# farshid83/dpsvm

Hardware: AMD Instinct MI355X
Metric: wall-clock training time (s) to tol=1e-3, MNIST even-odd RBF, at 1/2/4/8 MI355X (lower is better)
Workload: dtype fp32

## Files before the change

### dpsvm_amd/csrc/kernels/rbf_gemm_split.hip

```cpp
#include <hip/hip_runtime.h>

#include <algorithm>
#include <cmath>
#include <cstdlib>
#include <map>
#include <mutex>
#include <string>
#include <tuple>
#include <vector>

#include "dpsvm/common.hpp"
#include "device_util.hpp"
#include "kernels.hpp"
#include "split_mma.hpp"
#include "../runtime/hip_check.hpp"

namespace dpsvm {
namespace dev {

constexpr int kSplitThreads = 512;
constexpr int kSplitShiftTarget = 15;

constexpr int kSplitRowChunks = 4;
__global__ __launch_bounds__(256) void split_rows_kernel(const float* __restrict__ x, int64_t rows, int dp, int ldx,
                                                         u4* __restrict__ out, int32_t* __restrict__ shift,
                                                         int nkb) {
  const int lane = threadIdx.x & 63;
  const int64_t r = (int64_t)blockIdx.x * 4 + (threadIdx.x >> 6);
// ... 571 lines not shown
        o[7] = t;
      }
    }
    if (!has_next) break;
    L = Ln;
    t = tn_next;
    par ^= 1;
    Ln = L + G;
    if (Ln < ntiles) tn_next = tiles[Ln];
  }
}
#undef PIECE_A
#undef PIECE_B
#undef ROW_DMA

__device__ __forceinline__ bool h1_values(f16v (&H)[2][2], const float* s_sq, const int32_t* s_sh, const float* s_r,
                                          int lane, int wm, int wn, float gamma, float c0, float c1) {
  constexpr int TM = 256;
  const int hl = lane >> 5;
  const float ng = -gamma, l2e = 1.4426950408889634f;
  bool hot = false;
#pragma unroll
  for (int j = 0; j < 2; ++j) {
    const int cl = wn * 64 + 32 * j + (lane & 31);
    const float bsq = s_sq[TM + cl];
    const int nbsh = -s_sh[TM + cl];
    const float rb = s_r[TM + cl];
#pragma unroll
    for (int i = 0; i < 2; ++i) {
      __builtin_amdgcn_sched_barrier(0);
      const int lr0 = wm * 64 + 32 * i + 4 * hl;
#pragma unroll
      for (int g = 0; g < 4; ++g) {
        const f4 asq = *(const f4*)(s_sq + lr0 + 8 * g);
        const i4v ash = *(const i4v*)(s_sh + lr0 + 8 * g);
        const f4 ar = *(const f4*)(s_r + lr0 + 8 * g);
#pragma unroll
        for (int e = 0; e < 4; e += 2) {
          const int r = 4 * g + e;
          f2 h, dot, sq, d2, t;
          h.x = H[i][j][r];
          h.y = H[i][j][r + 1];
          {
#pragma clang fp contract(off)
            dot.x = ldexpf(h.x, nbsh - ash[e]);
            dot.y = ldexpf(h.y, nbsh - ash[e + 1]);
            sq.x = asq[e];
            sq.y = asq[e + 1];
            d2 = (sq + bsq) - (dot + dot);
            d2.x = d2.x > 0.f ? d2.x : 0.f;
            d2.y = d2.y > 0.f ? d2.y : 0.f;
            t = (ng * d2) * l2e;
            hot |= !split_cold(t.x, ar[e] + rb, c0, c1);
            hot |= !split_cold(t.y, ar[e + 1] + rb, c0, c1);
          }
          H[i][j][r] = __builtin_amdgcn_exp2f(t.x);
          H[i][j][r + 1] = __builtin_amdgcn_exp2f(t.y);
        }
      }
    }
  }
  return __builtin_amdgcn_ballot_w64(hot) != 0;
}

__device__ __forceinline__ void h1_store_block(const f16v& v, int i, int j, int lane, int wm, int wn, bool mirror,
                                               bool valid, float* out, int m0, int n0, int M, int N, int ldo) {
  constexpr int TM = 256, TN = 128;
  constexpr uint32_t OOB = 0x80000000u;
  const int hl = lane >> 5;
  float* const ob = out + ((int64_t)m0 * ldo + n0);
  float* const mb = out + ((int64_t)n0 * ldo + m0);
  const uint32_t ld = (uint32_t)ldo;
  const int rlim = min(M - m0, TM);
  const int clim = min(N - n0, TN);
  const int64_t ob_bytes = min<int64_t>((int64_t)(M - m0) * ldo * 4 - (int64_t)n0 * 4, (int64_t)OOB);
  const int64_t mb_bytes = min<int64_t>((int64_t)(N - n0) * ldo * 4 - (int64_t)m0 * 4, (int64_t)OOB);
  const __amdgpu_buffer_rsrc_t rs_o = __builtin_amdgcn_make_buffer_rsrc(ob, 0, (int)ob_bytes, 0x00020000);
  const __amdgpu_buffer_rsrc_t rs_m = __builtin_amdgcn_make_buffer_rsrc(mb, 0, (int)mb_bytes, 0x00020000);
  const int cl = wn * 64 + 32 * j + (lane & 31);
  const bool okc = valid && cl < clim;
  constexpr int CP = 0;
  const int lr0 = wm * 64 + 32 * i + 4 * hl;
// ... 16 lines not shown
    w.z = v[4 * q + 2];
    w.w = v[4 * q + 3];
    const uint32_t o = lr + 3 < rlim && okm ? vm + 32u * q : OOB;
    __builtin_amdgcn_raw_buffer_store_b128(__builtin_bit_cast(i4v, w), rs_m, (int)o, 0, CP);
    if (rlim < TM) {
#pragma unroll
      for (int c = 0; c < 4; ++c) {
        const uint32_t oc = (okm && lr + 3 >= rlim && lr + c < rlim) ? vm + 32u * q + 4u * c : OOB;
        const float vc = w[c];
        __builtin_amdgcn_raw_buffer_store_b32(__float_as_uint(vc), rs_m, (int)oc, 0, CP);
      }
    }
  }
}

__device__ __forceinline__ uint32_t clock_lo_v() {
  uint32_t c = (uint32_t)__builtin_amdgcn_s_memtime();
  asm volatile("" : "+v"(c));
  return c;
}

template <bool ST>
__device__ __noinline__ void h1s_dma(const u4* __restrict__ A, const int32_t* __restrict__ Ash,
                                     const float* __restrict__ Asq, const float* __restrict__ Ar, int M,
                                     const u4* __restrict__ B, const int32_t* __restrict__ Bsh,
                                     const float* __restrict__ Bsq, const float* __restrict__ Br, int N, int nst,
                                     const uint32_t* __restrict__ tiles, int ntiles, int L, int dwave, int lane,
                                     u4* lds, uint32_t* s_rows, uint64_t* stamps) {
  constexpr int TM = 256, TN = 128, ROWS = TM + TN, NB = 3, RD = 1536;
  const int G = gridDim.x;
  const uint32_t rs = (uint32_t)nst * 8;
  uint32_t t = tiles[L];
  int Ln = L + G;
  uint32_t tn_next = Ln < ntiles ? tiles[Ln] : 0u;
  uint32_t g = 0;
  const int dw = __builtin_amdgcn_readfirstlane(dwave);
    const int p = lane & 7;
    uint32_t off_e = 16u * ((uint32_t)(lane >> 3) * rs + (uint32_t)(p ^ (lane >> 4)));
    uint32_t off_o = 16u * ((uint32_t)(lane >> 3) * rs + (uint32_t)(p ^ ((lane >> 4) + 4)));
    asm volatile("" : "+v"(off_e), "+v"(off_o));
    auto stage = [&](int m0_, int n0_, int st, int buf) {
      const uint32_t uA = (uint32_t)(m0_ + 64 * dw) * rs + (uint32_t)st * 8;
      const uint32_t uB = (uint32_t)(n0_ + 32 * dw) * rs + (uint32_t)st * 8;
#pragma unroll
      for (int i = 0; i < 8; ++i) w64p_piece(A, lds, uA, 8 * rs, 64 * dw * 8, off_e, off_o, buf, i);
#pragma unroll
      for (int i = 0; i < 4; ++i) w64p_piece(B, lds, uB, 8 * rs, (TM + 32 * dw) * 8, off_e, off_o, buf, i);
    };
    const uint32_t* const rd_a =
        dw == 0 ? (const uint32_t*)Asq : dw == 1 ? (const uint32_t*)Ash : (const uint32_t*)Ar;
    const uint32_t* const rd_b =
        dw == 0 ? (const uint32_t*)Bsq : dw == 1 ? (const uint32_t*)Bsh : (const uint32_t*)Br;
    auto rowdata = [&](int m0_, int n0_, int par_) {
#pragma unroll
      for (int i = 0; i < 6; ++i) {
        const int r = 64 * i + lane;
        const int ri = i < 4 ? min(m0_ + r, M - 1) : min(n0_ + (r - TM), N - 1);
        const uint32_t* src = dw == 3 ? (const uint32_t*)Asq : (i < 4 ? rd_a : rd_b) + ri;
        lds_dma4(src, s_rows + par_ * RD + 64 * (6 * dw + i));
      }
    };
    {
      const int m0 = (int)(t >> 16) * TM, n0 = (int)(t & 0xffffu) * TN;
      stage(m0, n0, 0, 0);
      stage(m0, n0, 1, 1);
      rowdata(m0, n0, 0);
      asm volatile("s_waitcnt vmcnt(0)" ::: "memory");
    }
    int par = 0;
    while (true) {
      const bool has_next = Ln < ntiles;
      const int m0 = (int)(t >> 16) * TM, n0 = (int)(t & 0xffffu) * TN;
      const uint32_t tp = has_next ? tn_next : t;
      const int nm0 = (int)(tp >> 16) * TM, nn0 = (int)(tp & 0xffffu) * TN;
      uint32_t c_bar0 = 0, c_bar = 0, c_land = 0, c_t0 = 0;
      if constexpr (ST) c_t0 = clock_lo_v();
#pragma clang loop unroll(disable)
      for (int s = 0; s < nst; ++s) {
        uint32_t ca = 0, cb = 0;
        if constexpr (ST) ca = clock_lo_v();
        if (s == 1) asm volatile("s_waitcnt vmcnt(18)" ::: "memory");
        else asm volatile("s_waitcnt vmcnt(12)" ::: "memory");
        if constexpr (ST) cb = clock_lo_v();
        __builtin_amdgcn_s_barrier();
        asm volatile("" ::: "memory");
        if constexpr (ST) {
          const uint32_t cc = clock_lo_v();
          c_land += cb - ca;
          if (s == 0) c_bar0 = cc - cb;
          else c_bar += cc - cb;
        }
        const bool own = s + 2 < nst;
        stage(own ? m0 : nm0, own ? n0 : nn0, own ? s + 2 : s + 2 - nst, (int)((g + 2) % NB));
        if (s == 0) rowdata(nm0, nn0, par ^ 1);
        ++g;
      }
      if constexpr (ST) {
        const uint32_t c_t1 = clock_lo_v();
        if (dw == 0 && lane == 0) {
          uint64_t* o = stamps + (size_t)L * 16 + 8;
          o[0] = c_bar0;
          o[1] = c_bar;
          o[2] = c_land;
          o[3] = c_t1 - c_t0;
        }
      }
      if (!has_next) break;
      L = Ln;
      t = tn_next;
      par ^= 1;
      Ln = L + G;
      if (Ln < ntiles) tn_next = tiles[Ln];
    }
  asm volatile("s_waitcnt vmcnt(0)" ::: "memory");
}

constexpr int kH1sThreads = 768;
template <bool ST>
__global__ __launch_bounds__(kH1sThreads, 1) void rbf_gemm_split_h1s_kernel(
    const u4* __restrict__ A, const int32_t* __restrict__ Ash, const float* __restrict__ Asq,
    const float* __restrict__ Ar, int M, const u4* __restrict__ B, const int32_t* __restrict__ Bsh,
    const float* __restrict__ Bsq, const float* __restrict__ Br, int N, int nkb, float gamma, float c0, float c1,
    float* __restrict__ out, int ldo, int sym, const uint32_t* __restrict__ tiles, int ntiles,
    uint32_t* __restrict__ tile_hot, uint32_t* __restrict__ hot, uint64_t* __restrict__ stamps) {
  constexpr int WN = 2, TM = 256, TN = 128, ROWS = TM + TN, CPR = 8, BUF = ROWS * CPR, NB = 3, RD = 1536;
  __shared__ u4 lds[NB * BUF + 2 * RD / 4];
  uint32_t* const s_rows = (uint32_t*)(lds + NB * BUF);
  const int G = gridDim.x;
  int L = blockIdx.x;
  if (L >= ntiles) return;
  const int tid = threadIdx.x, lane = tid & 63, wave = tid >> 6;
  const int nst = (nkb + 1) >> 1;
  if (__builtin_amdgcn_readfirstlane(wave) >= 8) {
    h1s_dma<ST>(A, Ash, Asq, Ar, M, B, Bsh, Bsq, Br, N, nst, tiles, ntiles, L, wave - 8, lane, lds, s_rows, stamps);
    return;
  }
  uint32_t t = tiles[L];
  int Ln = L + G;
  uint32_t tn_next = Ln < ntiles ? tiles[Ln] : 0u;
  uint32_t g = 0;
  const int wm = wave / WN, wn = wave % WN, hl = lane >> 5;
  const int sw = ((lane & 31) >> 1) & 7;
  const int ra0 = (wm * 64 + (lane & 31)) * CPR;
  const int rb0 = (TM + wn * 64 + (lane & 31)) * CPR;
  int par = 0;
  auto stamp = [&](int i, uint32_t v) {
    if (tid == 0) stamps[(size_t)L * 16 + i] = v;
  };
  while (true) {
    const bool has_next = Ln < ntiles;
    const int tx = (int)(t >> 16), ty = (int)(t & 0xffffu);
    const int m0 = tx * TM, n0 = ty * TN;
    if constexpr (ST) {
      stamp(0, (uint32_t)__builtin_amdgcn_s_memtime());
      stamp(5, (uint32_t)__builtin_amdgcn_s_memrealtime());
    }
    f16v H[2][2];
#pragma unroll
    for (int i = 0; i < 2; ++i)
#pragma unroll
      for (int j = 0; j < 2; ++j)
#pragma unroll
        for (int r = 0; r < 16; ++r) H[i][j][r] = 0.f;
    auto stage = [&]<bool FS = false>() {
      ring_barrier();
      if constexpr (ST && FS) stamp(1, (uint32_t)__builtin_amdgcn_s_memtime());
      const u4* buf = lds + (g % NB) * BUF;
      const uint32_t abase = lds_addr(buf + ra0), bbase = lds_addr(buf + rb0);
      auto rd = [&](int q, h8& a0, h8& a1, h8& b0, h8& b1) {
        const uint32_t c = 16u * (uint32_t)((2 * q + hl) ^ sw);
        const uint32_t pa = abase + c, pb = bbase + c;
        asm volatile("ds_read_b128 %0, %1" : "=v"(a0) : "v"(pa) : "memory");
        asm volatile("ds_read_b128 %0, %1 offset:4096" : "=v"(a1) : "v"(pa) : "memory");
        asm volatile("ds_read_b128 %0, %1" : "=v"(b0) : "v"(pb) : "memory");
        asm volatile("ds_read_b128 %0, %1 offset:4096" : "=v"(b1) : "v"(pb) : "memory");
      };
      auto mma = [&](const h8& a0, const h8& a1, const h8& b0, const h8& b1) {
        H[0][0] = mfma32_f16(a0, b0, H[0][0]);
        H[0][1] = mfma32_f16(a0, b1, H[0][1]);
        H[1][0] = mfma32_f16(a1, b0, H[1][0]);
        H[1][1] = mfma32_f16(a1, b1, H[1][1]);
      };
      h8 x0, x1, x2, x3, y0, y1, y2, y3;
      rd(0, x0, x1, x2, x3);
      rd(1, y0, y1, y2, y3);
      asm volatile("s_waitcnt lgkmcnt(4)" : "+v"(x0), "+v"(x1), "+v"(x2), "+v"(x3));
      mma(x0, x1, x2, x3);
      rd(2, x0, x1, x2, x3);
      asm volatile("s_waitcnt lgkmcnt(4)" : "+v"(y0), "+v"(y1), "+v"(y2), "+v"(y3));
      mma(y0, y1, y2, y3);
      rd(3, y0, y1, y2, y3);
      asm volatile("s_waitcnt lgkmcnt(4)" : "+v"(x0), "+v"(x1), "+v"(x2), "+v"(x3));
      mma(x0, x1, x2, x3);
      asm volatile("s_waitcnt lgkmcnt(0)" : "+v"(y0), "+v"(y1), "+v"(y2), "+v"(y3));
      mma(y0, y1, y2, y3);
      ++g;
    };
    if constexpr (ST) stage.template operator()<true>();
#pragma clang loop unroll(disable)
    for (int s = ST ? 1 : 0; s < nst; ++s) stage();
    if constexpr (ST) stamp(2, (uint32_t)__builtin_amdgcn_s_memtime());
    int el = lane;
    asm volatile("" : "+v"(el));
    const float* rows = (const float*)(s_rows + par * RD);
    const bool hotw = h1_values(H, rows, (const int32_t*)(rows + ROWS), rows + 2 * ROWS, el, wm, wn, gamma, c0, c1);
    if constexpr (ST) stamp(3, (uint32_t)__builtin_amdgcn_s_memtime());
    const bool mirror = sym && ty > 2 * tx + (wm >> 1);
#pragma unroll
    for (int i = 0; i < 2; ++i)
#pragma unroll
      for (int j = 0; j < 2; ++j) {
        __builtin_amdgcn_sched_barrier(0);
        h1_store_block(H[i][j], i, j, el, wm, wn, mirror, true, out, m0, n0, M, N, ldo);
      }
    if (hotw && lane == 0) {
      if (atomicAdd(tile_hot + L, 1u) == 0u) {
        const uint32_t k = atomicAdd(hot, 1u);
        hot[1 + k] = t;
      }
    }
    if constexpr (ST) {
      stamp(4, (uint32_t)__builtin_amdgcn_s_memtime());
      stamp(6, (uint32_t)__builtin_amdgcn_s_memrealtime());
      stamp(7, t);
    }
    if (!has_next) break;
    L = Ln;
    t = tn_next;
    par ^= 1;
    Ln = L + G;
    if (Ln < ntiles) tn_next = tiles[Ln];
  }
  asm volatile("s_waitcnt vmcnt(0)" ::: "memory");
}

__global__ __launch_bounds__(256) void split_hplane_kernel(const u4* __restrict__ src, int64_t rows, int nkb,
                                                          u4* __restrict__ dst) {
  const int nq = ((nkb + 1) >> 1) * 8;
  const int64_t e = (int64_t)blockIdx.x * 256 + threadIdx.x;
  if (e >= rows * nq) return;
  const int64_t r = e / nq;
  const int q = (int)(e - r * nq), b = q >> 2, c = q & 3;
  dst[e] = b < nkb ? src[r * nkb * 8 + b * 8 + c] : u4{0u, 0u, 0u, 0u};
}

__global__ __launch_bounds__(256) void split_log2norm_kernel(const float* __restrict__ sq, int n,
                                                             float* __restrict__ r) {
  const int i = blockIdx.x * 256 + threadIdx.x;
  if (i < n) r[i] = split_log2norm(sq[i]);
}

}

namespace launch {

namespace {
int g_split_variant = -1;
}
// ... 54 lines not shown
  post_launch("split_rows_f16", s);
}

namespace {
struct TileTable {
  uint32_t* dev = nullptr;
  int64_t count = 0;
};
const TileTable& sym_tile_table(int64_t tm, int64_t tn, hipStream_t s, bool sym = true, bool one_product = false) {
  static std::mutex mu;
  static std::map<std::tuple<int, int64_t, int64_t, bool, bool>, TileTable> cache;
  const int device = current_device();
  std::lock_guard<std::mutex> lk(mu);
  auto it = cache.find({device, tm, tn, sym, one_product});
  if (it != cache.end()) return it->second;
  std::vector<uint32_t> order;
  const int64_t GM = one_product ? 8 : 4, CH = one_product ? 64 : 32;
  for (int64_t g0 = 0; g0 < tm; g0 += GM) {
    const int64_t gm = std::min(GM, tm - g0);
    for (int64_t ty = 0; ty < tn; ++ty)
      for (int64_t tx = g0; tx < g0 + gm; ++tx)
        if (!sym || ty >= 2 * tx) order.push_back((uint32_t)((tx << 16) | ty));
  }
  const int64_t total = (int64_t)order.size(), full = total / (8 * CH) * (8 * CH);
  std::vector<uint32_t> tab((size_t)total);
  for (int64_t L = 0; L < total; ++L) {
    int64_t T = L;
    if (L < full) {
      const int64_t xcd = L % 8, local = L / 8;
      T = ((local / CH) * 8 + xcd) * CH + local % CH;
    }
    tab[(size_t)L] = order[(size_t)T];
  }
  TileTable t;
  t.count = total;
  HIP_CHECK(hipMalloc((void**)&t.dev, (size_t)total * sizeof(uint32_t)));
  HIP_CHECK(hipMemcpyAsync(t.dev, tab.data(), (size_t)total * sizeof(uint32_t), hipMemcpyHostToDevice, s));
  HIP_CHECK(hipStreamSynchronize(s));
  return cache.emplace(std::make_tuple(device, tm, tn, sym, one_product), t).first->second;
}
}

void split_cold_consts(float gamma, float tau, float* c0, float* c1) {
  const double e = 4.5 * std::ldexp(1.0, -11) * (double)gamma;
  *c1 = (float)(-std::log2(e));
  *c0 = (float)(std::log2((double)tau) - std::log2(1.72 * e) - 0.01);
}

// ... 4 lines not shown

void gram_adapt_last(int64_t* tiles, int64_t* hot) {
  *tiles = t_adapt_tiles;
  *hot = t_adapt_tiles >= 0 && t_adapt_hot ? (int64_t)*(volatile uint32_t*)t_adapt_hot : -1;
}

void gram_adapt_prep(const void* A, const float* Asq, int64_t M, int dp, int64_t ldo, hipStream_t s,
                     GramAdaptPrep* prep) {
  *prep = GramAdaptPrep{};
  DPSVM_CHECK(M > 0 && split_gram_path(GramShape{M, M, ldo, dp, true, true}, split_gemm_variant()) ==
                           GramPath::Adaptive,
              "gram_adapt_prep: this Gram's plan is not adaptive");
  const int nkb = (dp + 31) / 32;
  const int64_t tm2 = (M + 255) / 256, tn = (M + 127) / 128;
  const int64_t ntiles = sym_tile_table(tm2, tn, s, true).count;
  const int64_t nq = (int64_t)((nkb + 1) / 2) * 8, ra = tm2 * 256;
  const size_t pb = (size_t)ra * nq * 16, rb = (size_t)M * 4, hb = (size_t)(2 * ntiles + 1) * 4;
  HIP_CHECK(hipMalloc(&prep->planes, pb));
  HIP_CHECK(hipMalloc((void**)&prep->r, rb));
  HIP_CHECK(hipMalloc((void**)&prep->hot, hb));
  prep->bytes = pb + rb + hb;
  dev::split_hplane_kernel<<<dim3((unsigned)((ra * nq + 255) / 256)), 256, 0, s>>>((const dev::u4*)A, ra, nkb,
                                                                                    (dev::u4*)prep->planes);
  post_launch("split_hplane", s);
  dev::split_log2norm_kernel<<<dim3((unsigned)((M + 255) / 256)), 256, 0, s>>>(Asq, (int)M, prep->r);
  post_launch("split_log2norm", s);
  prep->A = A;
  prep->M = M;
  prep->dp = dp;
  prep->ntiles = ntiles;
}

void gram_adapt_prep_free(GramAdaptPrep* prep) {
  if (prep->planes) (void)hipFree(prep->planes);
  if (prep->r) (void)hipFree(prep->r);
  if (prep->hot) (void)hipFree(prep->hot);
  *prep = GramAdaptPrep{};
}
// ... 51 lines not shown
void launch_gram_w64_persist(const GramArgs& g) {
  const int64_t tm2 = (g.M + 255) / 256, tn = (g.N + 127) / 128;
  const auto& t = sym_tile_table(tm2, tn, g.s, g.symmetric);
  const int64_t grid = std::min<int64_t>(t.count, persistent_grid_limit());
  auto pk = g_gram_stamps ? dev::rbf_gemm_split_w64p_kernel<true> : dev::rbf_gemm_split_w64p_kernel<false>;
  pk<<<dim3((unsigned)grid), dev::kW64Threads, 0, g.s>>>(
      (const dev::u4*)g.A, g.Ash, g.Asq, (int)g.M, (const dev::u4*)g.B, g.Bsh, g.Bsq, (int)g.N, g.nkb, g.gamma, g.out,
      (int)g.ldo, g.symmetric ? 1 : 0, t.dev, (int)t.count, (int)tm2, (int)tn, g_gram_stamps, nullptr, nullptr, 0.f,
      0.f, nullptr);
  post_launch("rbf_gemm_split_w64p", g.s);
}

void launch_gram_adaptive(const GramArgs& g, float cold_tau, const GramAdaptPrep* prep) {
  const int64_t tm2 = (g.M + 255) / 256, tn = (g.N + 127) / 128;
  const int64_t ntiles = sym_tile_table(tm2, tn, g.s, g.symmetric).count;
  const int64_t grid = std::min<int64_t>(ntiles, persistent_grid_limit());
  const auto& t1 = sym_tile_table(tm2, tn, g.s, g.symmetric, true);
  float c0 = 0.f, c1 = 0.f;
  split_cold_consts(g.gamma, cold_tau, &c0, &c1);
  const bool pre = prep && g.symmetric && prep->planes && prep->A == g.A && prep->M == g.M && prep->dp == g.dp &&
                   prep->ntiles == ntiles;
  const int64_t nr = g.symmetric ? g.M : g.M + g.N;
  float* r = pre ? prep->r : nullptr;
  uint32_t* hb = pre ? prep->hot : nullptr;
  if (!pre) {
    HIP_CHECK(hipMallocAsync((void**)&r, (size_t)nr * 4, g.s));
    HIP_CHECK(hipMallocAsync((void**)&hb, (size_t)(2 * ntiles + 1) * 4, g.s));
  }
  HIP_CHECK(hipMemsetAsync(hb, 0, (size_t)(ntiles + 1) * 4, g.s));
  float* br = r;
  if (!pre) {
    dev::split_log2norm_kernel<<<dim3((unsigned)((g.M + 255) / 256)), 256, 0, g.s>>>(g.Asq, (int)g.M, r);
    if (!g.symmetric) {
      br = r + g.M;
      dev::split_log2norm_kernel<<<dim3((unsigned)((g.N + 255) / 256)), 256, 0, g.s>>>(g.Bsq, (int)g.N, br);
    }
    post_launch("split_log2norm", g.s);
  }
  const void *hA = g.A, *hB = g.B;
  dev::u4* planes = nullptr;
  if (pre) {
    hA = hB = prep->planes;
  } else {
    const int64_t nq = (int64_t)((g.nkb + 1) / 2) * 8, ra = tm2 * 256, rb = g.symmetric ? 0 : tn * 128;
    HIP_CHECK(hipMallocAsync((void**)&planes, (size_t)(ra + rb) * nq * 16, g.s));
    dev::split_hplane_kernel<<<dim3((unsigned)((ra * nq + 255) / 256)), 256, 0, g.s>>>((const dev::u4*)g.A, ra, g.nkb,
                                                                                      planes);
    hA = hB = planes;
    if (!g.symmetric) {
      dev::split_hplane_kernel<<<dim3((unsigned)((rb * nq + 255) / 256)), 256, 0, g.s>>>((const dev::u4*)g.B, rb, g.nkb,
                                                                                        planes + ra * nq);
      hB = planes + ra * nq;
    }
    post_launch("split_hplane", g.s);
  }
  auto h1k = g_gram_stamps ? dev::rbf_gemm_split_h1s_kernel<true> : dev::rbf_gemm_split_h1s_kernel<false>;
  h1k<<<dim3((unsigned)grid), dev::kH1sThreads, 0, g.s>>>(
      (const dev::u4*)hA, g.Ash, g.Asq, r, (int)g.M, (const dev::u4*)hB, g.Bsh, g.Bsq, br, (int)g.N, g.nkb, g.gamma, c0,
      c1, g.out, (int)g.ldo, g.symmetric ? 1 : 0, t1.dev, (int)ntiles, hb, hb + ntiles, g_gram_stamps);
  if (planes) HIP_CHECK(hipFreeAsync(planes, g.s));
  post_launch("rbf_gemm_split_h1", g.s);
  dev::rbf_gemm_split_w64p_kernel<false, true><<<dim3((unsigned)grid), dev::kW64Threads, 0, g.s>>>(
      (const dev::u4*)g.A, g.Ash, g.Asq, (int)g.M, (const dev::u4*)g.B, g.Bsh, g.Bsq, (int)g.N, g.nkb, g.gamma, g.out,
      (int)g.ldo, g.symmetric ? 1 : 0, hb + ntiles + 1, 0, (int)tm2, (int)tn, nullptr, r, br, c0, c1, hb + ntiles);
  post_launch("rbf_gemm_split_w64p_hot", g.s);
  if (!t_adapt_hot) HIP_CHECK(hipHostMalloc((void**)&t_adapt_hot, 4, hipHostMallocDefault));
  HIP_CHECK(hipMemcpyAsync(t_adapt_hot, hb + ntiles, 4, hipMemcpyDeviceToHost, g.s));
  t_adapt_tiles = ntiles;
  if (!pre) {
    HIP_CHECK(hipFreeAsync(r, g.s));
    HIP_CHECK(hipFreeAsync(hb, g.s));
  }
}
}

void rbf_gemm_store_split(const void* A, const int32_t* Ash, const float* Asq, int64_t M, const void* B,
                          const int32_t* Bsh, const float* Bsq, int64_t N, int dp, float gamma, float* out,
                          int64_t ldo, hipStream_t s, bool symmetric, float cold_tau, const GramAdaptPrep* prep) {
  t_adapt_tiles = -1;
  if (M <= 0 || N <= 0) return;
  DPSVM_CHECK(!symmetric || (A == B && Asq == Bsq && Ash == Bsh && M == N && ldo % 4 == 0),
              "rbf_gemm_store_split: symmetric mode needs B == A, N == M");
// ... 16 lines not shown
```

### dpsvm_amd/csrc/python/bindings.cpp

```cpp
#include <pybind11/functional.h>
#include <pybind11/numpy.h>
#include <pybind11/pybind11.h>
#include <pybind11/stl.h>

#include "dpsvm/comm.hpp"
#include "dpsvm/common.hpp"
#include "dpsvm/device_state.hpp"
#include "dpsvm/io.hpp"
#include "dpsvm/solver.hpp"
#include "dpsvm/params_io.hpp"
#include "dpsvm/problem.hpp"
#include "dpsvm/ws_plan.hpp"
#include "../kernels/kernels.hpp"

namespace py = pybind11;
using namespace dpsvm;

namespace {

using F32 = py::array_t<float, py::array::c_style | py::array::forcecast>;

py::array_t<float> to_np(const std::vector<float>& v) {
  py::array_t<float> a((py::ssize_t)v.size());
  if (!v.empty()) memcpy(a.mutable_data(), v.data(), v.size() * 4);
  return a;
}
py::array_t<float> to_np2(const std::vector<float>& v, int64_t rows, int cols) {
// ... 906 lines not shown
                               uintptr_t stream, int reps) {
    return kernels::dot_gram_split((const float*)a, m_, (const float*)b, n, d, lda, ldb, dot_spec(kind, degree, coef0),
                                   gamma, (float*)out, out_ld, sym, (void*)stream, reps);
  }, py::arg("a"), py::arg("m"), py::arg("b"), py::arg("n"), py::arg("d"), py::arg("lda"), py::arg("ldb"),
     py::arg("kind"), py::arg("degree"), py::arg("coef0"), py::arg("gamma"), py::arg("out"), py::arg("out_ld"),
     py::arg("sym"), py::arg("stream"), py::arg("reps") = 0,
     "the Gram of a dot-product kernel (dot_gemm_split.hip) from f32 device rows; returns the event times (us) of "
     "reps launches before the returned one");
  m.def("split_cold_consts", [](float gamma, float tau) {
    float c0 = 0.f, c1 = 0.f;
    launch::split_cold_consts(gamma, tau, &c0, &c1);
    return py::make_tuple(c0, c1);
  }, "the adaptive Gram's element rule constants (c0, c1): cold iff R_i + R_j <= c1 and t1 <= c0 - (R_i + R_j)");
  m.def("k_gram_adapt_last", []() { return kernels::gram_adapt_last(); },
        "(one-product tiles, hot tiles) of the calling thread's last adaptive split Gram, or (-1, -1)");
  m.def("k_fused_select", [](uintptr_t f, uintptr_t alpha, uintptr_t y, int64_t n, float C, int rows, uintptr_t out,
                             uintptr_t stream) {
    kernels::fused_select((const float*)f, (const float*)alpha, (const float*)y, n, C, rows, (uint64_t*)out,
                          (void*)stream);
  });
  using U64 = py::array_t<uint64_t, py::array::c_style | py::array::forcecast>;
  using I32 = py::array_t<int32_t, py::array::c_style | py::array::forcecast>;
  auto vi = [](const I32& a) { return std::vector<int32_t>(a.data(), a.data() + a.size()); };
  m.def("k_ws_merge_multi", [vi](const U64& cand, int G, int blocks, int p_act, int q_max, int n_new, float eps,
                                 const I32& prev, int64_t iter, int64_t max_iter) {
    const auto r = kernels::ws_merge_multi_probe(std::vector<uint64_t>(cand.data(), cand.data() + cand.size()), G,
                                                 blocks, p_act, q_max, n_new, eps, vi(prev), iter, max_iter);
    py::dict d;
    d["uidx"] = r.uidx;
    d["idx"] = r.idx;
// ... 227 lines not shown
```

Measured before the change: 0.01569.

## Rework one-product RBF Gram pass to 256x256 tiles with unified DMA waves

Replaces the warp-specialized h1s kernel (8 compute waves plus 4 DMA waves, 256x128 tiles, 3-deep ring) with a 1024-thread kernel over 256x256 tiles. Every wave issues its own LDS DMA into a 4-deep ring with a new plane layout and swizzle. A new tile order groups 8 row tiles per column stripe and deals them across XCDs, and per-half hot flags feed the second hot-tile pass. The larger tile is meant to improve operand reuse and cut tile-loop overhead, at the cost of more LDS, a different plane layout, and dropping the timing-stamp instrumentation.

```diff
diff --git a/dpsvm_amd/csrc/kernels/gram_tile_order.hpp b/dpsvm_amd/csrc/kernels/gram_tile_order.hpp
--- /dev/null
+++ b/dpsvm_amd/csrc/kernels/gram_tile_order.hpp
@@ -0,0 +1,37 @@
+#pragma once
+#include <algorithm>
+#include <cstdint>
+#include <vector>
+
+namespace dpsvm {
+namespace launch {
+
+inline std::vector<uint32_t> xcd_deal(const std::vector<uint32_t>& order, int64_t CH) {
+  const int64_t total = (int64_t)order.size(), full = total / (8 * CH) * (8 * CH);
+  std::vector<uint32_t> tab((size_t)total);
+  for (int64_t L = 0; L < total; ++L) {
+    int64_t T = L;
+    if (L < full) {
+      const int64_t xcd = L % 8, local = L / 8;
+      T = ((local / CH) * 8 + xcd) * CH + local % CH;
+    }
+    tab[(size_t)L] = order[(size_t)T];
+  }
+  return tab;
+}
+
+inline std::vector<uint32_t> gram_tile_order(int64_t tm, int64_t tn, bool sym) {
+  constexpr int64_t GM = 8, CH = 32;
+  const int64_t tu = (tn + 1) / 2;
+  std::vector<uint32_t> order;
+  for (int64_t g0 = 0; g0 < tm; g0 += GM) {
+    const int64_t gm = std::min(GM, tm - g0);
+    for (int64_t u = 0; u < tu; ++u)
+      for (int64_t tx = g0; tx < g0 + gm; ++tx)
+        if (!sym || u >= tx) order.push_back((uint32_t)((tx << 16) | u));
+  }
+  return xcd_deal(order, CH);
+}
+
+}
+}
diff --git a/dpsvm_amd/csrc/kernels/rbf_gemm_split.hip b/dpsvm_amd/csrc/kernels/rbf_gemm_split.hip
--- a/dpsvm_amd/csrc/kernels/rbf_gemm_split.hip
+++ b/dpsvm_amd/csrc/kernels/rbf_gemm_split.hip
@@ -12,6 +12,7 @@
 #include "dpsvm/common.hpp"
 #include "device_util.hpp"
 #include "kernels.hpp"
+#include "gram_tile_order.hpp"
 #include "split_mma.hpp"
 #include "../runtime/hip_check.hpp"
 
@@ -613,58 +614,52 @@
 #undef PIECE_B
 #undef ROW_DMA
 
-__device__ __forceinline__ bool h1_values(f16v (&H)[2][2], const float* s_sq, const int32_t* s_sh, const float* s_r,
-                                          int lane, int wm, int wn, float gamma, float c0, float c1) {
+__device__ __forceinline__ bool h1_block_values(f16v& v, int i, int j, const float* s_sq, const int32_t* s_sh,
+                                                const float* s_r, int lane, int wm, int wn, float gamma, float c0,
+                                                float c1) {
   constexpr int TM = 256;
   const int hl = lane >> 5;
   const float ng = -gamma, l2e = 1.4426950408889634f;
   bool hot = false;
-#pragma unroll
-  for (int j = 0; j < 2; ++j) {
-    const int cl = wn * 64 + 32 * j + (lane & 31);
-    const float bsq = s_sq[TM + cl];
-    const int nbsh = -s_sh[TM + cl];
-    const float rb = s_r[TM + cl];
-#pragma unroll
-    for (int i = 0; i < 2; ++i) {
-      __builtin_amdgcn_sched_barrier(0);
-      const int lr0 = wm * 64 + 32 * i + 4 * hl;
-#pragma unroll
-      for (int g = 0; g < 4; ++g) {
-        const f4 asq = *(const f4*)(s_sq + lr0 + 8 * g);
-        const i4v ash = *(const i4v*)(s_sh + lr0 + 8 * g);
-        const f4 ar = *(const f4*)(s_r + lr0 + 8 * g);
-#pragma unroll
-        for (int e = 0; e < 4; e += 2) {
-          const int r = 4 * g + e;
-          f2 h, dot, sq, d2, t;
-          h.x = H[i][j][r];
-          h.y = H[i][j][r + 1];
-          {
+  const int cl = wn * 64 + 32 * j + (lane & 31);
+  const float bsq = s_sq[TM + cl];
+  const int nbsh = -s_sh[TM + cl];
+  const float rb = s_r[TM + cl];
+  const int lr0 = wm * 64 + 32 * i + 4 * hl;
+#pragma unroll
+  for (int g = 0; g < 4; ++g) {
+    const f4 asq = *(const f4*)(s_sq + lr0 + 8 * g);
+    const i4v ash = *(const i4v*)(s_sh + lr0 + 8 * g);
+    const f4 ar = *(const f4*)(s_r + lr0 + 8 * g);
+#pragma unroll
+    for (int e = 0; e < 4; e += 2) {
+      const int r = 4 * g + e;
+      f2 h, dot, sq, d2, t;
+      h.x = v[r];
+      h.y = v[r + 1];
+      {
 #pragma clang fp contract(off)
-            dot.x = ldexpf(h.x, nbsh - ash[e]);
-            dot.y = ldexpf(h.y, nbsh - ash[e + 1]);
-            sq.x = asq[e];
-            sq.y = asq[e + 1];
-            d2 = (sq + bsq) - (dot + dot);
-            d2.x = d2.x > 0.f ? d2.x : 0.f;
-            d2.y = d2.y > 0.f ? d2.y : 0.f;
-            t = (ng * d2) * l2e;
-            hot |= !split_cold(t.x, ar[e] + rb, c0, c1);
-            hot |= !split_cold(t.y, ar[e + 1] + rb, c0, c1);
-          }
-          H[i][j][r] = __builtin_amdgcn_exp2f(t.x);
-          H[i][j][r + 1] = __builtin_amdgcn_exp2f(t.y);
-        }
+        dot.x = ldexpf(h.x, nbsh - ash[e]);
+        dot.y = ldexpf(h.y, nbsh - ash[e + 1]);
+        sq.x = asq[e];
+        sq.y = asq[e + 1];
+        d2 = (sq + bsq) - (dot + dot);
+        d2.x = d2.x > 0.f ? d2.x : 0.f;
+        d2.y = d2.y > 0.f ? d2.y : 0.f;
+        t = (ng * d2) * l2e;
+        hot |= !split_cold(t.x, ar[e] + rb, c0, c1);
+        hot |= !split_cold(t.y, ar[e + 1] + rb, c0, c1);
       }
-    }
-  }
-  return __builtin_amdgcn_ballot_w64(hot) != 0;
+      v[r] = __builtin_amdgcn_exp2f(t.x);
+      v[r + 1] = __builtin_amdgcn_exp2f(t.y);
+    }
+  }
+  return hot;
 }
 
 __device__ __forceinline__ void h1_store_block(const f16v& v, int i, int j, int lane, int wm, int wn, bool mirror,
                                                bool valid, float* out, int m0, int n0, int M, int N, int ldo) {
-  constexpr int TM = 256, TN = 128;
+  constexpr int TM = 256, TN = 256;
   constexpr uint32_t OOB = 0x80000000u;
   const int hl = lane >> 5;
   float* const ob = out + ((int64_t)m0 * ldo + n0);
@@ -711,147 +706,75 @@
   }
 }
 
-__device__ __forceinline__ uint32_t clock_lo_v() {
-  uint32_t c = (uint32_t)__builtin_amdgcn_s_memtime();
-  asm volatile("" : "+v"(c));
-  return c;
-}
-
-template <bool ST>
-__device__ __noinline__ void h1s_dma(const u4* __restrict__ A, const int32_t* __restrict__ Ash,
-                                     const float* __restrict__ Asq, const float* __restrict__ Ar, int M,
-                                     const u4* __restrict__ B, const int32_t* __restrict__ Bsh,
-                                     const float* __restrict__ Bsq, const float* __restrict__ Br, int N, int nst,
-                                     const uint32_t* __restrict__ tiles, int ntiles, int L, int dwave, int lane,
-                                     u4* lds, uint32_t* s_rows, uint64_t* stamps) {
-  constexpr int TM = 256, TN = 128, ROWS = TM + TN, NB = 3, RD = 1536;
-  const int G = gridDim.x;
-  const uint32_t rs = (uint32_t)nst * 8;
-  uint32_t t = tiles[L];
-  int Ln = L + G;
-  uint32_t tn_next = Ln < ntiles ? tiles[Ln] : 0u;
-  uint32_t g = 0;
-  const int dw = __builtin_amdgcn_readfirstlane(dwave);
-    const int p = lane & 7;
-    uint32_t off_e = 16u * ((uint32_t)(lane >> 3) * rs + (uint32_t)(p ^ (lane >> 4)));
-    uint32_t off_o = 16u * ((uint32_t)(lane >> 3) * rs + (uint32_t)(p ^ ((lane >> 4) + 4)));
-    asm volatile("" : "+v"(off_e), "+v"(off_o));
-    auto stage = [&](int m0_, int n0_, int st, int buf) {
-      const uint32_t uA = (uint32_t)(m0_ + 64 * dw) * rs + (uint32_t)st * 8;
-      const uint32_t uB = (uint32_t)(n0_ + 32 * dw) * rs + (uint32_t)st * 8;
-#pragma unroll
-      for (int i = 0; i < 8; ++i) w64p_piece(A, lds, uA, 8 * rs, 64 * dw * 8, off_e, off_o, buf, i);
-#pragma unroll
-      for (int i = 0; i < 4; ++i) w64p_piece(B, lds, uB, 8 * rs, (TM + 32 * dw) * 8, off_e, off_o, buf, i);
-    };
-    const uint32_t* const rd_a =
-        dw == 0 ? (const uint32_t*)Asq : dw == 1 ? (const uint32_t*)Ash : (const uint32_t*)Ar;
-    const uint32_t* const rd_b =
-        dw == 0 ? (const uint32_t*)Bsq : dw == 1 ? (const uint32_t*)Bsh : (const uint32_t*)Br;
-    auto rowdata = [&](int m0_, int n0_, int par_) {
-#pragma unroll
-      for (int i = 0; i < 6; ++i) {
-        const int r = 64 * i + lane;
-        const int ri = i < 4 ? min(m0_ + r, M - 1) : min(n0_ + (r - TM), N - 1);
-        const uint32_t* src = dw == 3 ? (const uint32_t*)Asq : (i < 4 ? rd_a : rd_b) + ri;
-        lds_dma4(src, s_rows + par_ * RD + 64 * (6 * dw + i));
-      }
-    };
-    {
-      const int m0 = (int)(t >> 16) * TM, n0 = (int)(t & 0xffffu) * TN;
-      stage(m0, n0, 0, 0);
-      stage(m0, n0, 1, 1);
-      rowdata(m0, n0, 0);
-      asm volatile("s_waitcnt vmcnt(0)" ::: "memory");
-    }
-    int par = 0;
-    while (true) {
-      const bool has_next = Ln < ntiles;
-      const int m0 = (int)(t >> 16) * TM, n0 = (int)(t & 0xffffu) * TN;
-      const uint32_t tp = has_next ? tn_next : t;
-      const int nm0 = (int)(tp >> 16) * TM, nn0 = (int)(tp & 0xffffu) * TN;
-      uint32_t c_bar0 = 0, c_bar = 0, c_land = 0, c_t0 = 0;
-      if constexpr (ST) c_t0 = clock_lo_v();
-#pragma clang loop unroll(disable)
-      for (int s = 0; s < nst; ++s) {
-        uint32_t ca = 0, cb = 0;
-        if constexpr (ST) ca = clock_lo_v();
-        if (s == 1) asm volatile("s_waitcnt vmcnt(18)" ::: "memory");
-        else asm volatile("s_waitcnt vmcnt(12)" ::: "memory");
-        if constexpr (ST) cb = clock_lo_v();
-        __builtin_amdgcn_s_barrier();
-        asm volatile("" ::: "memory");
-        if constexpr (ST) {
-          const uint32_t cc = clock_lo_v();
-          c_land += cb - ca;
-          if (s == 0) c_bar0 = cc - cb;
-          else c_bar += cc - cb;
-        }
-        const bool own = s + 2 < nst;
-        stage(own ? m0 : nm0, own ? n0 : nn0, own ? s + 2 : s + 2 - nst, (int)((g + 2) % NB));
-        if (s == 0) rowdata(nm0, nn0, par ^ 1);
-        ++g;
-      }
-      if constexpr (ST) {
-        const uint32_t c_t1 = clock_lo_v();
-        if (dw == 0 && lane == 0) {
-          uint64_t* o = stamps + (size_t)L * 16 + 8;
-          o[0] = c_bar0;
-          o[1] = c_bar;
-          o[2] = c_land;
-          o[3] = c_t1 - c_t0;
-        }
-      }
-      if (!has_next) break;
-      L = Ln;
-      t = tn_next;
-      par ^= 1;
-      Ln = L + G;
-      if (Ln < ntiles) tn_next = tiles[Ln];
-    }
-  asm volatile("s_waitcnt vmcnt(0)" ::: "memory");
-}
-
-constexpr int kH1sThreads = 768;
-template <bool ST>
-__global__ __launch_bounds__(kH1sThreads, 1) void rbf_gemm_split_h1s_kernel(
+template <class T>
+__device__ __forceinline__ T pick(bool c, T a, T b) {
+  return c ? a : b;
+}
+
+constexpr int kH1Threads = 1024;
+__global__ __launch_bounds__(kH1Threads, 1) void rbf_gemm_split_h1_kernel(
     const u4* __restrict__ A, const int32_t* __restrict__ Ash, const float* __restrict__ Asq,
-    const float* __restrict__ Ar, int M, const u4* __restrict__ B, const int32_t* __restrict__ Bsh,
-    const float* __restrict__ Bsq, const float* __restrict__ Br, int N, int nkb, float gamma, float c0, float c1,
-    float* __restrict__ out, int ldo, int sym, const uint32_t* __restrict__ tiles, int ntiles,
-    uint32_t* __restrict__ tile_hot, uint32_t* __restrict__ hot, uint64_t* __restrict__ stamps) {
-  constexpr int WN = 2, TM = 256, TN = 128, ROWS = TM + TN, CPR = 8, BUF = ROWS * CPR, NB = 3, RD = 1536;
+    const float* __restrict__ Ar, int M, int RA, const u4* __restrict__ B, const int32_t* __restrict__ Bsh,
+    const float* __restrict__ Bsq, const float* __restrict__ Br, int N, int RB, int nst, float gamma, float c0,
+    float c1, float* __restrict__ out, int ldo, int sym, const uint32_t* __restrict__ tiles, int ntiles, int tn,
+    uint32_t* __restrict__ half_hot, uint32_t* __restrict__ hot) {
+  constexpr int WN = 4, TM = 256, TN = 256, ROWS = TM + TN, CPR = 4, BUF = ROWS * CPR, NB = 4, RD = 2048;
   __shared__ u4 lds[NB * BUF + 2 * RD / 4];
   uint32_t* const s_rows = (uint32_t*)(lds + NB * BUF);
   const int G = gridDim.x;
   int L = blockIdx.x;
   if (L >= ntiles) return;
   const int tid = threadIdx.x, lane = tid & 63, wave = tid >> 6;
-  const int nst = (nkb + 1) >> 1;
-  if (__builtin_amdgcn_readfirstlane(wave) >= 8) {
-    h1s_dma<ST>(A, Ash, Asq, Ar, M, B, Bsh, Bsq, Br, N, nst, tiles, ntiles, L, wave - 8, lane, lds, s_rows, stamps);
-    return;
-  }
+  const int wv = __builtin_amdgcn_readfirstlane(wave);
+  const int wm = wave / WN, wn = wave % WN, hl = lane >> 5;
+  const bool a_wave = wv < 8;
+  const u4* const P = pick(a_wave, A, B);
+  const int64_t R = pick(a_wave, RA, RB);
+  const int prow = a_wave ? 32 * wv : 32 * (wv - 8);
+  uint32_t loff = 16u * (uint32_t)((lane >> 2) * 4 + ((lane & 3) ^ ((lane >> 4) & 3)));
+  asm volatile("" : "+v"(loff));
+  auto stage_dma = [&](int m0_, int n0_, int st, int buf) {
+    const char* src = (const char*)(P + ((int64_t)st * R + pick(a_wave, m0_, n0_) + prow) * CPR);
+    u4* dst = lds + buf * BUF + 32 * wv * CPR;
+    lds_dma16(src + loff, dst);
+    lds_dma16(src + 1024 + loff, dst + 16 * CPR);
+  };
+  auto rowdata = [&](int m0_, int n0_, int par_) {
+#pragma unroll
+    for (int i = 0; i < 2; ++i) {
+      const int q = wv + 16 * i, ch = q & 7;
+      const bool a_rows = ch < 4, pad = q >= 24;
+      const float* const fa = pick(q < 8 || pad, Asq, Ar);
+      const float* const fb = pick(pad, Asq, pick(q < 8, Bsq, Br));
+      const uint32_t* base = pick(q >= 8 && q < 16, (const uint32_t*)pick(a_rows, Ash, Bsh),
+                                  (const uint32_t*)pick(a_rows, fa, fb));
+      const int r = 64 * (ch & 3) + lane;
+      const int ri = pad ? min(lane, M - 1) : a_rows ? min(m0_ + r, M - 1) : min(n0_ + r, N - 1);
+      lds_dma4(base + ri, s_rows + par_ * RD + 64 * q);
+    }
+  };
   uint32_t t = tiles[L];
   int Ln = L + G;
   uint32_t tn_next = Ln < ntiles ? tiles[Ln] : 0u;
   uint32_t g = 0;
-  const int wm = wave / WN, wn = wave % WN, hl = lane >> 5;
-  const int sw = ((lane & 31) >> 1) & 7;
-  const int ra0 = (wm * 64 + (lane & 31)) * CPR;
-  const int rb0 = (TM + wn * 64 + (lane & 31)) * CPR;
+  {
+    const int m0 = (int)(t >> 16) * TM, n0 = (int)(t & 0xffffu) * TN;
+    rowdata(m0, n0, 0);
+    stage_dma(m0, n0, 0, 0);
+    stage_dma(m0, n0, 1, 1);
+    stage_dma(m0, n0, 2, 2);
+    asm volatile("s_waitcnt vmcnt(0)" ::: "memory");
+  }
+  const int sw = (lane >> 2) & 3;
+  const uint32_t ra0 = (uint32_t)(wm * 64 + (lane & 31)) * 64u, rb0 = (uint32_t)(TM + wn * 64 + (lane & 31)) * 64u;
+  const uint32_t ck0 = 16u * (uint32_t)(hl ^ sw), ck1 = 16u * (uint32_t)((2 + hl) ^ sw);
   int par = 0;
-  auto stamp = [&](int i, uint32_t v) {
-    if (tid == 0) stamps[(size_t)L * 16 + i] = v;
-  };
   while (true) {
     const bool has_next = Ln < ntiles;
-    const int tx = (int)(t >> 16), ty = (int)(t & 0xffffu);
-    const int m0 = tx * TM, n0 = ty * TN;
-    if constexpr (ST) {
-      stamp(0, (uint32_t)__builtin_amdgcn_s_memtime());
-      stamp(5, (uint32_t)__builtin_amdgcn_s_memrealtime());
-    }
+    const int tx = (int)(t >> 16), tu = (int)(t & 0xffffu);
+    const int m0 = tx * TM, n0 = tu * TN;
+    const uint32_t tp = has_next ? tn_next : t;
+    const int nm0 = (int)(tp >> 16) * TM, nn0 = (int)(tp & 0xffffu) * TN;
     f16v H[2][2];
 #pragma unroll
     for (int i = 0; i < 2; ++i)
@@ -859,68 +782,61 @@
       for (int j = 0; j < 2; ++j)
 #pragma unroll
         for (int r = 0; r < 16; ++r) H[i][j][r] = 0.f;
-    auto stage = [&]<bool FS = false>() {
+#pragma clang loop unroll(disable)
+    for (int s = 0; s < nst; ++s) {
+      asm volatile("s_waitcnt vmcnt(4)" ::: "memory");
       ring_barrier();
-      if constexpr (ST && FS) stamp(1, (uint32_t)__builtin_amdgcn_s_memtime());
-      const u4* buf = lds + (g % NB) * BUF;
-      const uint32_t abase = lds_addr(buf + ra0), bbase = lds_addr(buf + rb0);
-      auto rd = [&](int q, h8& a0, h8& a1, h8& b0, h8& b1) {
-        const uint32_t c = 16u * (uint32_t)((2 * q + hl) ^ sw);
-        const uint32_t pa = abase + c, pb = bbase + c;
-        asm volatile("ds_read_b128 %0, %1" : "=v"(a0) : "v"(pa) : "memory");
-        asm volatile("ds_read_b128 %0, %1 offset:4096" : "=v"(a1) : "v"(pa) : "memory");
-        asm volatile("ds_read_b128 %0, %1" : "=v"(b0) : "v"(pb) : "memory");
-        asm volatile("ds_read_b128 %0, %1 offset:4096" : "=v"(b1) : "v"(pb) : "memory");
-      };
-      auto mma = [&](const h8& a0, const h8& a1, const h8& b0, const h8& b1) {
-        H[0][0] = mfma32_f16(a0, b0, H[0][0]);
-        H[0][1] = mfma32_f16(a0, b1, H[0][1]);
-        H[1][0] = mfma32_f16(a1, b0, H[1][0]);
-        H[1][1] = mfma32_f16(a1, b1, H[1][1]);
+      const bool own = s + 3 < nst;
+      stage_dma(own ? m0 : nm0, own ? n0 : nn0, own ? s + 3 : s + 3 - nst, (int)((g + 3) % NB));
+      const uint32_t bb = lds_addr(lds + (g % NB) * BUF);
+      const uint32_t pa = bb + ra0, pb = bb + rb0;
+      auto rd = [&](uint32_t c, h8& a0, h8& a1, h8& b0, h8& b1) {
+        const uint32_t qa = pa + c, qb = pb + c;
+        asm volatile("ds_read_b128 %0, %1" : "=v"(a0) : "v"(qa) : "memory");
+        asm volatile("ds_read_b128 %0, %1 offset:2048" : "=v"(a1) : "v"(qa) : "memory");
+        asm volatile("ds_read_b128 %0, %1" : "=v"(b0) : "v"(qb) : "memory");
+        asm volatile("ds_read_b128 %0, %1 offset:2048" : "=v"(b1) : "v"(qb) : "memory");
       };
       h8 x0, x1, x2, x3, y0, y1, y2, y3;
-      rd(0, x0, x1, x2, x3);
-      rd(1, y0, y1, y2, y3);
+      rd(ck0, x0, x1, x2, x3);
+      rd(ck1, y0, y1, y2, y3);
       asm volatile("s_waitcnt lgkmcnt(4)" : "+v"(x0), "+v"(x1), "+v"(x2), "+v"(x3));
-      mma(x0, x1, x2, x3);
-      rd(2, x0, x1, x2, x3);
-      asm volatile("s_waitcnt lgkmcnt(4)" : "+v"(y0), "+v"(y1), "+v"(y2), "+v"(y3));
-      mma(y0, y1, y2, y3);
-      rd(3, y0, y1, y2, y3);
-      asm volatile("s_waitcnt lgkmcnt(4)" : "+v"(x0), "+v"(x1), "+v"(x2), "+v"(x3));
-      mma(x0, x1, x2, x3);
+      H[0][0] = mfma32_f16(x0, x2, H[0][0]);
+      H[0][1] = mfma32_f16(x0, x3, H[0][1]);
+      H[1][0] = mfma32_f16(x1, x2, H[1][0]);
+      H[1][1] = mfma32_f16(x1, x3, H[1][1]);
+      __builtin_amdgcn_sched_barrier(0);
       asm volatile("s_waitcnt lgkmcnt(0)" : "+v"(y0), "+v"(y1), "+v"(y2), "+v"(y3));
-      mma(y0, y1, y2, y3);
+      H[0][0] = mfma32_f16(y0, y2, H[0][0]);
+      H[0][1] = mfma32_f16(y0, y3, H[0][1]);
+      H[1][0] = mfma32_f16(y1, y2, H[1][0]);
+      H[1][1] = mfma32_f16(y1, y3, H[1][1]);
       ++g;
-    };
-    if constexpr (ST) stage.template operator()<true>();
-#pragma clang loop unroll(disable)
-    for (int s = ST ? 1 : 0; s < nst; ++s) stage();
-    if constexpr (ST) stamp(2, (uint32_t)__builtin_amdgcn_s_memtime());
+    }
+    if (has_next) rowdata(nm0, nn0, par ^ 1);
     int el = lane;
     asm volatile("" : "+v"(el));
     const float* rows = (const float*)(s_rows + par * RD);
-    const bool hotw = h1_values(H, rows, (const int32_t*)(rows + ROWS), rows + 2 * ROWS, el, wm, wn, gamma, c0, c1);
-    if constexpr (ST) stamp(3, (uint32_t)__builtin_amdgcn_s_memtime());
-    const bool mirror = sym && ty > 2 * tx + (wm >> 1);
-#pragma unroll
-    for (int i = 0; i < 2; ++i)
-#pragma unroll
-      for (int j = 0; j < 2; ++j) {
+    const bool mirror = sym && tu > tx;
+    bool hotw = false;
+#pragma unroll
+    for (int j = 0; j < 2; ++j)
+#pragma unroll
+      for (int i = 0; i < 2; ++i) {
+        __builtin_amdgcn_sched_barrier(0);
+        hotw |= __builtin_amdgcn_ballot_w64(h1_block_values(H[i][j], i, j, rows, (const int32_t*)(rows + ROWS),
+                                                            rows + 2 * ROWS, el, wm, wn, gamma, c0, c1)) != 0;
         __builtin_amdgcn_sched_barrier(0);
         h1_store_block(H[i][j], i, j, el, wm, wn, mirror, true, out, m0, n0, M, N, ldo);
       }
-    if (hotw && lane == 0) {
-      if (atomicAdd(tile_hot + L, 1u) == 0u) {
+    const int half = wn >> 1, ty = 2 * tu + half;
+    if (hotw && ty < tn && lane == 0) {
+      if (atomicAdd(half_hot + 2 * L + half, 1u) == 0u) {
         const uint32_t k = atomicAdd(hot, 1u);
-        hot[1 + k] = t;
+        hot[1 + k] = ((uint32_t)tx << 16) | (uint32_t)ty;
       }
     }
-    if constexpr (ST) {
-      stamp(4, (uint32_t)__builtin_amdgcn_s_memtime());
-      stamp(6, (uint32_t)__builtin_amdgcn_s_memrealtime());
-      stamp(7, t);
-    }
+    asm volatile("s_waitcnt vmcnt(0)" ::: "memory");
     if (!has_next) break;
     L = Ln;
     t = tn_next;
@@ -928,17 +844,15 @@
     Ln = L + G;
     if (Ln < ntiles) tn_next = tiles[Ln];
   }
-  asm volatile("s_waitcnt vmcnt(0)" ::: "memory");
 }
 
 __global__ __launch_bounds__(256) void split_hplane_kernel(const u4* __restrict__ src, int64_t rows, int nkb,
                                                           u4* __restrict__ dst) {
-  const int nq = ((nkb + 1) >> 1) * 8;
   const int64_t e = (int64_t)blockIdx.x * 256 + threadIdx.x;
-  if (e >= rows * nq) return;
-  const int64_t r = e / nq;
-  const int q = (int)(e - r * nq), b = q >> 2, c = q & 3;
-  dst[e] = b < nkb ? src[r * nkb * 8 + b * 8 + c] : u4{0u, 0u, 0u, 0u};
+  if (e >= rows * nkb * 4) return;
+  const int64_t b = e / (rows * 4), q = e - b * rows * 4, r = q >> 2;
+  const int c = (int)(q & 3);
+  dst[e] = src[r * nkb * 8 + b * 8 + c];
 }
 
 __global__ __launch_bounds__(256) void split_log2norm_kernel(const float* __restrict__ sq, int n,
@@ -1023,24 +937,21 @@
   std::lock_guard<std::mutex> lk(mu);
   auto it = cache.find({device, tm, tn, sym, one_product});
   if (it != cache.end()) return it->second;
-  std::vector<uint32_t> order;
-  const int64_t GM = one_product ? 8 : 4, CH = one_product ? 64 : 32;
-  for (int64_t g0 = 0; g0 < tm; g0 += GM) {
-    const int64_t gm = std::min(GM, tm - g0);
-    for (int64_t ty = 0; ty < tn; ++ty)
-      for (int64_t tx = g0; tx < g0 + gm; ++tx)
-        if (!sym || ty >= 2 * tx) order.push_back((uint32_t)((tx << 16) | ty));
-  }
-  const int64_t total = (int64_t)order.size(), full = total / (8 * CH) * (8 * CH);
-  std::vector<uint32_t> tab((size_t)total);
-  for (int64_t L = 0; L < total; ++L) {
-    int64_t T = L;
-    if (L < full) {
-      const int64_t xcd = L % 8, local = L / 8;
-      T = ((local / CH) * 8 + xcd) * CH + local % CH;
-    }
-    tab[(size_t)L] = order[(size_t)T];
-  }
+  std::vector<uint32_t> tab;
+  if (one_product) {
+    tab = gram_tile_order(tm, tn, sym);
+  } else {
+    std::vector<uint32_t> order;
+    const int64_t GM = 4, CH = 32;
+    for (int64_t g0 = 0; g0 < tm; g0 += GM) {
+      const int64_t gm = std::min(GM, tm - g0);
+      for (int64_t ty = 0; ty < tn; ++ty)
+        for (int64_t tx = g0; tx < g0 + gm; ++tx)
+          if (!sym || ty >= 2 * tx) order.push_back((uint32_t)((tx << 16) | ty));
+    }
+    tab = xcd_deal(order, CH);
+  }
+  const int64_t total = (int64_t)tab.size();
   TileTable t;
   t.count = total;
   HIP_CHECK(hipMalloc((void**)&t.dev, (size_t)total * sizeof(uint32_t)));
@@ -1075,14 +986,15 @@
   const int nkb = (dp + 31) / 32;
   const int64_t tm2 = (M + 255) / 256, tn = (M + 127) / 128;
   const int64_t ntiles = sym_tile_table(tm2, tn, s, true).count;
-  const int64_t nq = (int64_t)((nkb + 1) / 2) * 8, ra = tm2 * 256;
-  const size_t pb = (size_t)ra * nq * 16, rb = (size_t)M * 4, hb = (size_t)(2 * ntiles + 1) * 4;
+  const int64_t nt256 = sym_tile_table(tm2, tn, s, true, true).count;
+  const int64_t ra = tm2 * 256, np = ra * nkb * 4;
+  const size_t pb = (size_t)np * 16, rb = (size_t)M * 4, hb = (size_t)(2 * nt256 + 1 + ntiles) * 4;
   HIP_CHECK(hipMalloc(&prep->planes, pb));
   HIP_CHECK(hipMalloc((void**)&prep->r, rb));
   HIP_CHECK(hipMalloc((void**)&prep->hot, hb));
   prep->bytes = pb + rb + hb;
-  dev::split_hplane_kernel<<<dim3((unsigned)((ra * nq + 255) / 256)), 256, 0, s>>>((const dev::u4*)A, ra, nkb,
-                                                                                    (dev::u4*)prep->planes);
+  dev::split_hplane_kernel<<<dim3((unsigned)((np + 255) / 256)), 256, 0, s>>>((const dev::u4*)A, ra, nkb,
+                                                                             (dev::u4*)prep->planes);
   post_launch("split_hplane", s);
   dev::split_log2norm_kernel<<<dim3((unsigned)((M + 255) / 256)), 256, 0, s>>>(Asq, (int)M, prep->r);
   post_launch("split_log2norm", s);
@@ -1164,8 +1076,10 @@
 void launch_gram_adaptive(const GramArgs& g, float cold_tau, const GramAdaptPrep* prep) {
   const int64_t tm2 = (g.M + 255) / 256, tn = (g.N + 127) / 128;
   const int64_t ntiles = sym_tile_table(tm2, tn, g.s, g.symmetric).count;
-  const int64_t grid = std::min<int64_t>(ntiles, persistent_grid_limit());
   const auto& t1 = sym_tile_table(tm2, tn, g.s, g.symmetric, true);
+  const int64_t nt256 = t1.count;
+  const int64_t grid1 = std::min<int64_t>(nt256, persistent_grid_limit());
+  const int64_t grid2 = std::min<int64_t>(ntiles, persistent_grid_limit());
   float c0 = 0.f, c1 = 0.f;
   split_cold_consts(g.gamma, cold_tau, &c0, &c1);
   const bool pre = prep && g.symmetric && prep->planes && prep->A == g.A && prep->M == g.M && prep->dp == g.dp &&
@@ -1175,9 +1089,10 @@
   uint32_t* hb = pre ? prep->hot : nullptr;
   if (!pre) {
     HIP_CHECK(hipMallocAsync((void**)&r, (size_t)nr * 4, g.s));
-    HIP_CHECK(hipMallocAsync((void**)&hb, (size_t)(2 * ntiles + 1) * 4, g.s));
-  }
-  HIP_CHECK(hipMemsetAsync(hb, 0, (size_t)(ntiles + 1) * 4, g.s));
+    HIP_CHECK(hipMallocAsync((void**)&hb, (size_t)(2 * nt256 + 1 + ntiles) * 4, g.s));
+  }
+  HIP_CHECK(hipMemsetAsync(hb, 0, (size_t)(2 * nt256 + 1) * 4, g.s));
+  uint32_t* const hot = hb + 2 * nt256;
   float* br = r;
   if (!pre) {
     dev::split_log2norm_kernel<<<dim3((unsigned)((g.M + 255) / 256)), 256, 0, g.s>>>(g.Asq, (int)g.M, r);
@@ -1187,35 +1102,35 @@
     }
     post_launch("split_log2norm", g.s);
   }
-  const void *hA = g.A, *hB = g.B;
+  const int64_t ra = tm2 * 256, rb = g.symmetric ? ra : (g.N + 255) / 256 * 256;
+  const dev::u4 *hA = nullptr, *hB = nullptr;
   dev::u4* planes = nullptr;
   if (pre) {
-    hA = hB = prep->planes;
+    hA = hB = (const dev::u4*)prep->planes;
   } else {
-    const int64_t nq = (int64_t)((g.nkb + 1) / 2) * 8, ra = tm2 * 256, rb = g.symmetric ? 0 : tn * 128;
-    HIP_CHECK(hipMallocAsync((void**)&planes, (size_t)(ra + rb) * nq * 16, g.s));
-    dev::split_hplane_kernel<<<dim3((unsigned)((ra * nq + 255) / 256)), 256, 0, g.s>>>((const dev::u4*)g.A, ra, g.nkb,
-                                                                                      planes);
+    const int64_t npa = ra * g.nkb * 4, npb = g.symmetric ? 0 : rb * g.nkb * 4;
+    HIP_CHECK(hipMallocAsync((void**)&planes, (size_t)(npa + npb) * 16, g.s));
+    dev::split_hplane_kernel<<<dim3((unsigned)((npa + 255) / 256)), 256, 0, g.s>>>((const dev::u4*)g.A, ra, g.nkb,
+                                                                                  planes);
     hA = hB = planes;
     if (!g.symmetric) {
-      dev::split_hplane_kernel<<<dim3((unsigned)((rb * nq + 255) / 256)), 256, 0, g.s>>>((const dev::u4*)g.B, rb, g.nkb,
-                                                                                        planes + ra * nq);
-      hB = planes + ra * nq;
+      dev::split_hplane_kernel<<<dim3((unsigned)((npb + 255) / 256)), 256, 0, g.s>>>((const dev::u4*)g.B, rb, g.nkb,
+                                                                                    planes + npa);
+      hB = planes + npa;
     }
     post_launch("split_hplane", g.s);
   }
-  auto h1k = g_gram_stamps ? dev::rbf_gemm_split_h1s_kernel<true> : dev::rbf_gemm_split_h1s_kernel<false>;
-  h1k<<<dim3((unsigned)grid), dev::kH1sThreads, 0, g.s>>>(
-      (const dev::u4*)hA, g.Ash, g.Asq, r, (int)g.M, (const dev::u4*)hB, g.Bsh, g.Bsq, br, (int)g.N, g.nkb, g.gamma, c0,
-      c1, g.out, (int)g.ldo, g.symmetric ? 1 : 0, t1.dev, (int)ntiles, hb, hb + ntiles, g_gram_stamps);
+  dev::rbf_gemm_split_h1_kernel<<<dim3((unsigned)grid1), dev::kH1Threads, 0, g.s>>>(
+      hA, g.Ash, g.Asq, r, (int)g.M, (int)ra, hB, g.Bsh, g.Bsq, br, (int)g.N, (int)rb, g.nkb, g.gamma, c0, c1, g.out,
+      (int)g.ldo, g.symmetric ? 1 : 0, t1.dev, (int)nt256, (int)tn, hb, hot);
   if (planes) HIP_CHECK(hipFreeAsync(planes, g.s));
   post_launch("rbf_gemm_split_h1", g.s);
-  dev::rbf_gemm_split_w64p_kernel<false, true><<<dim3((unsigned)grid), dev::kW64Threads, 0, g.s>>>(
+  dev::rbf_gemm_split_w64p_kernel<false, true><<<dim3((unsigned)grid2), dev::kW64Threads, 0, g.s>>>(
       (const dev::u4*)g.A, g.Ash, g.Asq, (int)g.M, (const dev::u4*)g.B, g.Bsh, g.Bsq, (int)g.N, g.nkb, g.gamma, g.out,
-      (int)g.ldo, g.symmetric ? 1 : 0, hb + ntiles + 1, 0, (int)tm2, (int)tn, nullptr, r, br, c0, c1, hb + ntiles);
+      (int)g.ldo, g.symmetric ? 1 : 0, hot + 1, 0, (int)tm2, (int)tn, nullptr, r, br, c0, c1, hot);
   post_launch("rbf_gemm_split_w64p_hot", g.s);
   if (!t_adapt_hot) HIP_CHECK(hipHostMalloc((void**)&t_adapt_hot, 4, hipHostMallocDefault));
-  HIP_CHECK(hipMemcpyAsync(t_adapt_hot, hb + ntiles, 4, hipMemcpyDeviceToHost, g.s));
+  HIP_CHECK(hipMemcpyAsync(t_adapt_hot, hot, 4, hipMemcpyDeviceToHost, g.s));
   t_adapt_tiles = ntiles;
   if (!pre) {
     HIP_CHECK(hipFreeAsync(r, g.s));
diff --git a/dpsvm_amd/csrc/python/bindings.cpp b/dpsvm_amd/csrc/python/bindings.cpp
--- a/dpsvm_amd/csrc/python/bindings.cpp
+++ b/dpsvm_amd/csrc/python/bindings.cpp
@@ -11,6 +11,7 @@
 #include "dpsvm/params_io.hpp"
 #include "dpsvm/problem.hpp"
 #include "dpsvm/ws_plan.hpp"
+#include "../kernels/gram_tile_order.hpp"
 #include "../kernels/kernels.hpp"
 
 namespace py = pybind11;
@@ -947,6 +948,10 @@
   }, "the adaptive Gram's element rule constants (c0, c1): cold iff R_i + R_j <= c1 and t1 <= c0 - (R_i + R_j)");
   m.def("k_gram_adapt_last", []() { return kernels::gram_adapt_last(); },
         "(one-product tiles, hot tiles) of the calling thread's last adaptive split Gram, or (-1, -1)");
+  m.def("gram_tile_order", [](int64_t tm, int64_t tn, bool sym) { return launch::gram_tile_order(tm, tn, sym); },
+        py::arg("tm"), py::arg("tn"), py::arg("sym"),
+        "the one-product Gram pass's table of 256 x 256 tiles, entries (tx << 16) | u, for tm 256-row tiles by tn "
+        "128-column tiles, in the order the persistent workgroups walk it (host only)");
   m.def("k_fused_select", [](uintptr_t f, uintptr_t alpha, uintptr_t y, int64_t n, float C, int rows, uintptr_t out,
                              uintptr_t stream) {
     kernels::fused_select((const float*)f, (const float*)alpha, (const float*)y, n, C, rows, (uint64_t*)out,
```

After: 0.01511 (median of 6 runs). 3.7% less time.
